# fishaudio/Bert-VITS2

Measured on AMD Instinct MI355X. Metric: audio-seconds/sec (44.1 kHz), SynthesizerTrn.infer(), 128-phoneme utterance, higher is better.
Workload: dtype f32; 1 GPU; BASELINE config 2: B=1 x T=128 symbols per GPU, fp32 Generator (split-bf16 MFMA), fp32 flow, fp32 text encoder / durations / spline; utterances_per_gpu=1, symbols=128, frames=384, parallelism=utterance-sharded x1, hipgraph=False, hip_force_dev_kernarg=1

## Files before the change

bert-vits2_amd/build.py:

```python
from __future__ import annotations

import hashlib
import os
import shutil
import subprocess
import sys

HERE = os.path.dirname(os.path.realpath(__file__))
CSRC = os.path.join(HERE, "csrc")
ROOT = os.path.dirname(HERE)
LIB = os.path.join(CSRC, "libbv2.so")
STAMP = os.path.join(CSRC, ".libbv2.stamp")

SOURCES = [
    "bv2_api.cpp", "bv2_model.cpp", "bv2_exec.cpp", "bv2_bert.cpp",
    "kernels/conv_mfma.hip", "kernels/conv_x6.hip", "kernels/respair_x6.hip", "kernels/resblock_fused.hip", "kernels/gen_bf16.hip", "kernels/resblock_cl_bf16.hip", "kernels/resblock_c16_bf16.hip", "kernels/respair_cl_bf16.hip", "kernels/enc_f16.hip", "kernels/layernorm.hip", "kernels/attention.hip", "kernels/misc.hip", "kernels/dds_fused.hip", "kernels/flow_boundary.hip", "kernels/bert.hip", "kernels/deberta_attn.hip", "kernels/ref_enc.hip", "kernels/stft.hip", "kernels/stream.hip",
]
EXPORTS = "libbv2.map"
HEADERS = [EXPORTS, "bv2_internal.h", "bv2_kernels.h", "kernels/spline.h", "kernels/cl_bf16.h", os.path.join(ROOT, "include", "bv2.h"),
           os.path.join(ROOT, "include", "bv2_testing.h"), os.path.join(ROOT, "include", "bv2_bert.h")]
FLAGS = ["--offload-arch=gfx950", "-O3", "-std=c++17", "-fPIC", "-Wall", "-Wno-unused-function", "-x", "hip"]


def _hipcc() -> str:
    for c in (os.environ.get("HIPCC"), shutil.which("hipcc"), "/opt/rocm/bin/hipcc"):
        if c and os.path.exists(c):
            return c
    raise RuntimeError("hipcc not found (need ROCm's hipcc to build libbv2.so for gfx950)")


def _digest() -> str:
# ... 53 lines not shown
```

bert-vits2_amd/csrc/bv2_api.cpp:

```cpp
#include <cmath>
#include <cstddef>
#include <cstring>
#include <functional>
#include <new>

#include "bv2_internal.h"

using namespace bv2;

static thread_local std::string g_create_err;

#define BV2_TRY try {
#define BV2_CATCH(h_)                                                                  \
  } catch (const std::exception& e) {                                                  \
    if (h_) (h_)->err = std::string("exception: ") + e.what();                         \
    return -100;                                                                       \
  } catch (...) {                                                                      \
    if (h_) (h_)->err = "unknown exception";                                           \
    return -100;                                                                       \
  }

extern "C" {

int bv2_abi_version(void) { return BV2_ABI_VERSION; }
// ... 28 lines not shown
  } catch (...) {
    delete h;
    g_create_err = "bv2_create: out of memory";
    return -100;
  }
  *out = h;
  return 0;
}

void bv2_destroy(bv2_handle* h) {
  if (!h) return;
  for (auto& r : h->prof_pool) { (void)hipEventDestroy(r.e0); (void)hipEventDestroy(r.e1); }
  if (h->ev_fork) (void)hipEventDestroy(h->ev_fork);
  if (h->ev_join) (void)hipEventDestroy(h->ev_join);
  if (h->side_stream) (void)hipStreamDestroy(h->side_stream);
  delete h;
}

const char* bv2_last_error(const bv2_handle* h) { return h ? h->err.c_str() : g_create_err.c_str(); }

static float half_to_float(uint16_t v) {
  const uint32_t sign = (uint32_t)(v & 0x8000) << 16;
  uint32_t exp = (v >> 10) & 0x1f, man = v & 0x3ff, bits;
  if (exp == 0) {
    if (man == 0) bits = sign;
    else {
      exp = 127 - 15 + 1;
      while (!(man & 0x400)) { man <<= 1; --exp; }
      man &= 0x3ff;
      bits = sign | (exp << 23) | (man << 13);
// ... 44 lines not shown
  uint32_t hdr[8];
  if (hipMemcpy(hdr, dev_blob, sizeof(hdr), hipMemcpyDeviceToHost) != hipSuccess) {
    h->err = "bv2_attach_weights: cannot read the blob header (is this a device pointer on the current GPU?)";
    return -6;
  }
  int64_t tf;
  std::memcpy(&tf, hdr + 4, sizeof(tf));
  if (hdr[0] != kBlobMagic || hdr[1] != BV2_ABI_VERSION || hdr[2] != h->model.cfg_hash || tf != h->model.total_floats) {
    h->err = "bv2_attach_weights: blob header does not match this handle's config (not packed, or packed for another model)";
    return -7;
  }
  if (hdr[3] != BV2_PACK_LAYOUT) {
    h->err = "bv2_attach_weights: blob was packed with another pack layout (a cache written by an older library build): repack";
    return -7;
  }
  h->blob = static_cast<const float*>(dev_blob);
  return 0;
  BV2_CATCH(h)
}

int bv2_detach_weights(bv2_handle* h) {
  if (!h) return -1;
  h->blob = nullptr;
  return 0;
}

int bv2_set_generator_dtype(bv2_handle* h, int dtype) {
  if (!h) return -1;
  if (dtype != BV2_F32 && dtype != BV2_BF16) { h->err = "bv2_set_generator_dtype: BV2_F32 or BV2_BF16"; return -1; }
  if (dtype == BV2_BF16) {
    const Model& m = h->model;
    bool ok = m.conv_pre.wb_off >= 0 && m.post_c % 8 == 0 && m.post_c <= 64;
    for (int i = 0; i < m.n_ups && ok; ++i) {
      ok = m.ups[i].cl.wb_off >= 0 && conv_cl_bf16_supported(m.ups[i].cl.cin, m.ups[i].cl.cout, m.ups[i].cl.k, 1);
      for (int j = 0; j < m.n_rbk && ok; ++j)
        for (int d = 0; d < m.n_rbd && ok; ++d)
          ok = m.rb[i][j][d][0].wb_off >= 0 &&
               conv_cl_bf16_supported(m.rb[i][j][d][0].cin, m.rb[i][j][d][0].cout, m.rb[i][j][d][0].k,
// ... 508 lines not shown
  if (!g) return;
  if (g->exec) (void)hipGraphExecDestroy(g->exec);
  delete g;
}

int bv2_set_option(bv2_handle* h, const char* key, int value) {
  if (!h) return -1;
  BV2_TRY
  const std::string k = key ? key : "";
  if (k == "fused_resblock") h->no_fused_resblock = value == 0;
  else if (k == "fused_respair") h->no_fused_respair = value == 0;
  else if (k == "fused_boundary") h->no_fused_boundary = value == 0;
  else if (k == "x6_pair") h->no_x6_pair = value == 0;
  else if (k == "x6_pair_c64") h->no_x6_pair_c64 = value == 0;
  else if (k == "x6_pair_c16") h->no_x6_pair_c16 = value == 0;
  else if (k == "x6_pair_c128") h->x6_pair_c128 = value != 0;
  else if (k == "respair_mix") h->respair_problem_major = value == 0;
  else if (k == "respair_form") h->respair_form = value;
  else if (k == "respair_c32") h->no_respair_c32 = value == 0;
  else if (k == "f16_wn") h->f16_wn = value;
  else if (k == "f16_ni") h->f16_ni = value;
  else if (k == "f16_kv") h->no_f16_kv = !value;
  else if (k == "stage_sum") h->no_stage_sum = !value;
  else if (k == "resblock_c16") h->no_resblock_c16 = value == 0;
  else if (k == "f16_fused_ln") h->no_f16_fused_ln = value == 0;
  else if (k == "f16_ksplit") h->no_f16_ksplit = value == 0;
  else if (k == "conv_post_rows") h->no_conv_post_rows = value == 0;
  else if (k == "ups_phase_taps") h->no_ups_phase_taps = value == 0;
  else if (k == "xcd_affine") h->no_xcd_affine = value == 0;
  else if (k == "prefetch") h->prefetch = value & 3;
// ... 385 lines not shown
    if (hipMemset(base, 0, boff + pb.size() * 4) != hipSuccess) return -6;
    if (hipMemcpy(base, pk.data(), pk.size() * 2, hipMemcpyHostToDevice) != hipSuccess) return -6;
    if (hipMemcpy(base + boff, pb.data(), pb.size() * 4, hipMemcpyHostToDevice) != hipSuccess) return -6;
    FusedLaunch F;
    std::memset(&F, 0, sizeof(F));
    F.nprob = 1; F.B = B; F.C = C; F.L = L; F.slope = slope; F.lens = lens; F.len_mul = 1;
    FusedProb& q = F.p[0];
    q.x = x; q.out = out; q.k = k; q.dil = dil;
    q.w61 = reinterpret_cast<const uint16_t*>(base); q.w62 = q.w61 + ne;
    q.b1 = reinterpret_cast<const float*>(base + boff); q.b2 = q.b1 + cout_pad;
    q.w1 = q.b1; q.w2 = q.b1;
    return launch_respair_x6(static_cast<hipStream_t>(stream), F);
  } catch (...) { return -100; }
}

int bv2_test_flow_boundary(void* stream, const float* a, int nslab, int64_t slab_stride, const float* gamma, const float* beta,
                           const float* mask, float* x1, int64_t z_bstride, const float* post_w_host, const float* post_b_host,
                           const float* pre_w_host, const float* pre_b_host, float* pre_out, float* wpack_dev, int B, int C, int T) {
  try {
    const int C1 = C / 2;
    const size_t npost = (size_t)t_round_up(C, 16) * t_round_up(C1, 128), npre = (size_t)t_round_up(C1, 16) * t_round_up(C, 128);
    std::vector<float> pk(npost + npre + (size_t)C1 + (size_t)C + 64, 0.f);
    for (int co = 0; co < C1; ++co)
      for (int ci = 0; ci < C; ++ci) pk[(size_t)conv_w_index(0, ci, co, t_round_up(C, 16), 1)] = post_w_host[(size_t)co * C + ci];
    if (pre_w_host)
      for (int co = 0; co < C; ++co)
        for (int ci = 0; ci < C1; ++ci) pk[npost + (size_t)conv_w_index(0, ci, co, t_round_up(C1, 16), 1)] = pre_w_host[(size_t)co * C1 + ci];
    for (int co = 0; co < C1; ++co) pk[npost + npre + co] = post_b_host[co];
    if (pre_b_host)
      for (int co = 0; co < C; ++co) pk[npost + npre + C1 + co] = pre_b_host[co];
// ... 253 lines not shown
```

bert-vits2_amd/csrc/bv2_exec.cpp:

```cpp
#include <cmath>
#include <cstdlib>
#include <cstring>

#include "bv2_internal.h"

namespace bv2 {

namespace {

struct Arena {
  char* base;
  int64_t off = 0, cap;
  Arena(void* b, int64_t c) : base(static_cast<char*>(b)), cap(c) {}
  template <class T> T* get(int64_t n) {
    const int64_t bytes = (n * (int64_t)sizeof(T) + 255) / 256 * 256;
    T* p = base ? reinterpret_cast<T*>(base + off) : nullptr;
    off += bytes;
    return p;
  }
  bool ok() const { return base == nullptr || off <= cap; }
};

struct Ctx {
  bv2_handle* h;
// ... 789 lines not shown
      hres = P.outacc;
    }
    {
      const std::string tn = "flow." + std::to_string(a) + ".enc";
      c.tap(tn.c_str(), hres, (int64_t)B * H * Ty);
    }
    p = c.prob(K.post, hres, x1, Ty);
    p.out_bstride = (int64_t)C * Ty; p.res = x1; p.res_bstride = (int64_t)C * Ty; p.res_mode = RES_RSUB;
    p.out_mask = ymask; p.mask_post = 1;
    c.conv1(p, B, Ty, "flow.post");
    {
      const std::string tn = "flow." + std::to_string(a) + ".z";
      c.tap(tn.c_str(), z, (int64_t)B * C * Ty);
    }
  }
}

static void gen_core(Ctx& c, const PlanB& P, const float* z, int z_rstride, const float* ymask, int B, int L, float* o,
                     const int64_t* lens) {
  const Model& m = c.m;
  const bv2_config& cf = m.cfg;
  const int C = cf.inter_channels, c0 = cf.upsample_initial_channel;
  {
    ConvProb p = c.prob(m.conv_pre, z, P.pre, L);
    p.x_bstride = (int64_t)C * z_rstride; p.x_rstride = z_rstride; p.Lin = L;
    p.in_mask = ymask; p.in_mask_bstride = z_rstride;
    p.bias2 = P.gv; p.bias2_bstride = P.gv_stride;
    c.conv1(p, B, L, "dec.conv_pre", 1, 0, lens, 1);
  }
  c.tap("dec.pre", P.pre, (int64_t)B * c0 * L);
// ... 57 lines not shown
        const bool to_cur = ((m.n_rbd - 1 - d) & 1) == 0;
        for (int jj = 0; jj < nb; ++jj) {
          const int j = nb - 1 - jj;
          float* cur = S[1 + j];
          float* tmp = S[1 + nb + j];
          const float* xin = d == 0 ? x : (to_cur ? tmp : cur);
          ConvProb p = c.prob(m.rb[i][j][d][0], xin, to_cur ? cur : tmp, Lo, cf.resblock_dilation_sizes[j][d]);
          p.pre_act = PRE_LRELU; p.slope = 0.1f;
          p.res = xin; p.res_mode = RES_ADD;
          p.w6 = (!c.h->no_conv_x6 && m.rb[i][j][d][0].wx_off >= 0) ? reinterpret_cast<const uint16_t*>(c.W(m.rb[i][j][d][0].wx_off)) : nullptr;
          c1.p[jj] = p;
        }
        c.conv(c1, "dec.resblock2.conv");
      }
      for (int j = 0; j < nb; ++j) branch_out[j] = S[1 + j];
    } else if (fused) {
      for (int j = 0; j < nb; ++j) branch_out[j] = nullptr;
      for (int d = 0; d < m.n_rbd; ++d) {
        FusedLaunch F;
        std::memset(&F, 0, sizeof(F));
        F.nprob = nb; F.B = B; F.C = U.cout; F.L = Lo; F.slope = 0.1f; F.lens = lens; F.len_mul = up * U.u;
        for (int jj = 0; jj < nb; ++jj) {
          const int j = nb - 1 - jj;
          float* a = S[1 + j];
          float* b2 = S[1 + nb + j];
          const float* xin = d == 0 ? x : branch_out[j];
          float* xout = (xin == a) ? b2 : a;
          FusedProb& p = F.p[jj];
          p.x = xin; p.out = xout;
          p.w1 = c.W(m.rb[i][j][d][0].w_off); p.b1 = c.W(m.rb[i][j][d][0].b_off);
// ... 487 lines not shown
```

bert-vits2_amd/csrc/bv2_internal.h:

```cpp
#pragma once
#include <hip/hip_runtime_api.h>
#include <stdint.h>

#include <map>
#include <string>
#include <vector>

#include "../../include/bv2.h"
#include "bv2_kernels.h"

namespace bv2 {

constexpr int kAttnWindow = 4;
constexpr int kCondLayer = 2;
constexpr int kSdpLayers = 3;
constexpr int kSdpKernel = 3;
constexpr int kSdpBins = 10;
constexpr int kSdpFlowsUsed = 3;
constexpr int kDpFilter = 256;
constexpr int kDpKernel = 3;
constexpr int kFlowKernel = 5;
constexpr int kMaxLayers = 16;
constexpr int kMaxFlows = 8;
constexpr uint32_t kBlobMagic = 0x32765642u;
// ... 65 lines not shown
  VecW dp_g1, dp_b1, dp_g2, dp_b2;
  VecW emb_g;
  RefEncW ref_enc;
  int n_coupling = 0;
  CouplingW coupling[kMaxFlows];
  ConvW conv_pre;
  GemvW dec_cond;
  int n_ups = 0, n_rbk = 0, n_rbd = 0;
  int rb_type = 1;
  UpW ups[BV2_MAX_UPS];
  ConvW rb[BV2_MAX_UPS][BV2_MAX_RESBLOCK_KERNELS][BV2_MAX_RESBLOCK_DILATIONS][2];
  int64_t rbcl_w_off[BV2_MAX_UPS][BV2_MAX_RESBLOCK_KERNELS];
  int64_t rbcl_b_off[BV2_MAX_UPS][BV2_MAX_RESBLOCK_KERNELS];
  int64_t rb16_w_off[BV2_MAX_UPS][BV2_MAX_RESBLOCK_KERNELS];
  int64_t rb16_b_off[BV2_MAX_UPS][BV2_MAX_RESBLOCK_KERNELS];
  VecW conv_post;
  int post_c = 0, post_k = 7;
  int total_up = 1;
  int64_t total_floats = 0;
  uint32_t cfg_hash = 0;
};

struct HostTensor { std::vector<float> data; std::vector<int64_t> shape; };

struct ProfileRec { hipEvent_t e0, e1; int fam; double flops, bytes; };

struct Tap { float* dst; int64_t cap; };

}

struct bv2_handle {
  bv2::Model model;
  std::map<std::string, bv2::HostTensor> tensors;
  const float* blob = nullptr;
  std::string err;
  std::map<std::string, bv2::Tap> taps;
  int gen_dtype = BV2_F32;
  int flow_dtype = BV2_F32;
  bool no_conv_x6 = false;
  bool no_conv_x3 = false;
  bool x6_narrow = true;
  bool no_fused_resblock = false;
  int prefetch = 0;
  bool no_xcd_affine = false;
  bool no_f16_fused_ln = false;
  int f16_wn = 0, f16_ni = 0;
  bool no_f16_kv = false;
  bool no_f16_ksplit = false;
  bool no_conv_post_rows = false;
  bool no_ups_phase_taps = false;
  bool no_stage_sum = true;
  bool no_resblock_c16 = false;
  bool no_respair_c32 = false;
  int respair_form = 1;
  bool respair_problem_major = false;
  bool x6_pair_c128 = false;
  bool no_x6_pair_c16 = false;
  bool no_x6_pair_c64 = false;
  bool no_x6_pair = false;
  bool no_fused_boundary = false;
  bool no_fused_respair = false;
  bool no_fused_attn_o = false;
  int attn_ksplit = -1;
  bool no_fused_dds = false;
  bool no_overlap_dp = true;
  hipStream_t side_stream = nullptr;
  hipEvent_t ev_fork = nullptr, ev_join = nullptr;
  bool prof_on = false;
  int prof_mode = 1;
  std::vector<bv2::ProfileRec> prof_pool;
  size_t prof_used = 0;
  std::vector<std::string> prof_names;
};

namespace bv2 {

int build_layout(Model& m, std::string& err);
int pack_blob(const Model& m, const std::map<std::string, HostTensor>& t, float* blob, std::string& err);
bool key_in_schema(const Model& m, const std::string& key);

int64_t workspace_bytes(const Model& m, int B, int T, int Ty);
int run_encode(bv2_handle* h, hipStream_t s, const bv2_encode_in& in, const bv2_encode_out& out, void* ws, int64_t wsb,
               const bv2_item_controls* ic = nullptr, const float* g_in = nullptr);
int run_ref_encode(bv2_handle* h, hipStream_t s, const float* y, const int64_t* strides, const int64_t* y_lengths, int B, int L,
                   float* g_out, void* ws, int64_t wsb);
int run_decode(bv2_handle* h, hipStream_t s, const bv2_decode_in& in, const bv2_decode_out& out, void* ws, int64_t wsb,
               const bv2_item_controls* ic = nullptr);
int run_flow(bv2_handle* h, hipStream_t s, int B, int Ty, const float* z_p, const int64_t* y_lengths, const float* y_mask,
             const float* g, float* z, void* ws, int64_t wsb);
int run_stage_emb_g(bv2_handle* h, hipStream_t s, int B, const int64_t* sid, float* g);
int run_stage_enc_p(bv2_handle* h, hipStream_t s, int B, int T, const int64_t* x, const int64_t* tone, const int64_t* lang,
                    const float* b0, const float* b1, const float* b2, const float* g, const int64_t* x_lengths, float* xout,
                    float* m_p, float* logs_p, float* x_mask, void* ws, int64_t wsb);
int run_stage_sdp(bv2_handle* h, hipStream_t s, int B, int T, const float* x, const float* x_mask, const float* zin,
// ... 14 lines not shown
```

bert-vits2_amd/csrc/bv2_kernels.h:

```cpp
#pragma once
#include <hip/hip_runtime_api.h>
#include <stdint.h>
#include <map>
#include <mutex>
#include <utility>

namespace bv2 {

#if defined(__HIPCC__)
__device__ __forceinline__ bool xcd_decode(unsigned id, int per, int B, int& b, int& r) {
  const unsigned slot = id >> 3;
  b = (int)(slot / (unsigned)per) * 8 + (int)(id & 7u);
  r = (int)(slot % (unsigned)per);
  return b < B;
}
#endif
inline int xcd_grid(int B, int per) { return 8 * ((B + 7) / 8) * per; }

struct Prefetch { const void* ptr; unsigned bytes; };
constexpr int PF_BLOCKS = 128;
#if defined(__HIPCC__)
__device__ __forceinline__ void prefetch_tail(const Prefetch pf, unsigned l, unsigned j, unsigned tid, unsigned nthreads) {
  const unsigned lines = (pf.bytes + 127u) >> 7;
  const unsigned lx = (lines + 7u) >> 3;
// ... 142 lines not shown
  const float* w1; const float* b1;
  const float* w2; const float* b2;
  int k, dil;
  const uint16_t* w61; const uint16_t* w62;
  const uint16_t* w31; const uint16_t* w32;
  const float* w3inv1; const float* w3inv2;
};
struct FusedLaunch { FusedProb p[3]; int nprob, B, C, L; float slope; const int64_t* lens = nullptr; int len_mul = 1;
                     unsigned long long* dbg = nullptr; };
bool resblock_fused_supported(int C, int k, int dil);
int launch_resblock_fused(hipStream_t stream, const FusedLaunch& F);
double resblock_fused_flops(const FusedLaunch& F);
double resblock_fused_bytes(const FusedLaunch& F);
bool respair_x6_supported(int C, int k, int dil);
int launch_respair_x6(hipStream_t stream, const FusedLaunch& F);

struct ClProb {
  const uint16_t* x[3];
  int nsrc; float in_scale;
  int64_t x_bstride;
  int Lin;
  const uint16_t* w;
  const float* bias;
  const float* bias2;
  int bias2_bstride;
  uint16_t* out;
  int64_t out_bstride;
  const uint16_t* res;
  int64_t res_bstride;
  int cin, cout, cout_pad, k, dil, pad_left;
// ... 297 lines not shown
```

bert-vits2_amd/csrc/bv2_model.cpp:

```cpp
#include <cmath>
#include <cstddef>
#include <cstring>
#include <functional>

#include "bv2_internal.h"

namespace bv2 {

static inline int round_up(int x, int m) { return (x + m - 1) / m * m; }

static inline uint16_t f2bf(float f) {
  uint32_t u;
  std::memcpy(&u, &f, 4);
  if ((u & 0x7fffffffu) > 0x7f800000u) return (uint16_t)((u >> 16) | 0x40u);
  u += 0x7fffu + ((u >> 16) & 1u);
  return (uint16_t)(u >> 16);
}

static inline uint16_t f2h(float f) {
  const _Float16 h = (_Float16)f;
  uint16_t u;
  std::memcpy(&u, &h, 2);
  return u;
}
// ... 311 lines not shown
          const float v = w[((int64_t)co * cin + ci) * 9 + t];
          if (i == 0) dst[t * 32 + co] = v;
          else dst[(((int64_t)(co / 8) * cin + ci) * 9 + t) * 8 + co % 8] = v;
        }
  }
  const int K = 128 * W[6];
  R.w_ih = P.vec("ref_enc.gru.weight_ih_l0", {384, K});
  R.w_hh = P.vec("ref_enc.gru.weight_hh_l0", {384, 128});
  R.b_ih = P.vec("ref_enc.gru.bias_ih_l0", {384});
  R.b_hh = P.vec("ref_enc.gru.bias_hh_l0", {384});
  R.pw = P.vec("ref_enc.proj.weight", {c.gin_channels, 128});
  R.pb = P.vec("ref_enc.proj.bias", {c.gin_channels});
}

int pack_all(Model& m, Packer& P) {
  const bv2_config& c = m.cfg;
  const int hid = c.hidden_channels, inter = c.inter_channels, filt = c.filter_channels, gin = c.gin_channels;
  const int half = inter / 2;

  m.emb = P.vec("enc_p.emb.weight", {c.n_vocab, hid});
  m.tone_emb = P.vec("enc_p.tone_emb.weight", {c.n_tones, hid});
  m.lang_emb = P.vec("enc_p.language_emb.weight", {c.n_languages, hid});
  const char* bn[3] = {"enc_p.bert_proj", "enc_p.ja_bert_proj", "enc_p.en_bert_proj"};
  for (int i = 0; i < 3; ++i) m.bert[i] = P.conv1d(bn[i], hid, c.bert_dim, 1);
  m.enc = pack_encoder(P, "enc_p.encoder", hid, filt, c.n_heads, c.n_layers, c.kernel_size, gin);
  m.proj_m = P.conv1d("enc_p.proj", 2 * inter, hid, 1, true, false, 0, inter);
  m.proj_logs = P.conv1d("enc_p.proj", 2 * inter, hid, 1, true, false, inter, inter);

  m.sdp_pre = P.conv1d("sdp.pre", hid, hid, 1);
  m.sdp_proj = P.conv1d("sdp.proj", hid, hid, 1);
// ... 111 lines not shown
      const std::string rp = "dec.resblocks." + std::to_string(i * m.n_rbk + j);
      P.emit_x6 = ch >= 16 && ch % 16 == 0;
      const bool rb2 = c.resblock_type == 2;
      for (int d = 0; d < m.n_rbd; ++d) {
        if (rb2) {
          m.rb[i][j][d][0] = P.conv1d(rp + ".convs." + std::to_string(d), ch, ch, k, true, true);
          m.rb[i][j][d][1] = ConvW();
        } else {
          m.rb[i][j][d][0] = P.conv1d(rp + ".convs1." + std::to_string(d), ch, ch, k, true, true);
          m.rb[i][j][d][1] = P.conv1d(rp + ".convs2." + std::to_string(d), ch, ch, k, true, true);
        }
      }
      P.emit_x6 = false;
      if (rb2) {
        m.rbcl_w_off[i][j] = m.rbcl_b_off[i][j] = m.rb16_w_off[i][j] = m.rb16_b_off[i][j] = -1;
        continue;
      }
      m.rbcl_w_off[i][j] = m.rbcl_b_off[i][j] = -1;
      if (m.n_rbd <= BV2_RBCL_MAX_D && resblock_cl_bf16_supported(ch, k, c.resblock_dilation_sizes[j], m.n_rbd)) {
        const int U = (ch / 16) * k, Upad = resblock_cl_bf16_units(ch, k);
        m.rbcl_w_off[i][j] = P.alloc(((int64_t)(2 * m.n_rbd * Upad + RBCL_PD) * 512 + 1) / 2);
        m.rbcl_b_off[i][j] = P.alloc((int64_t)2 * m.n_rbd * 32);
        if (P.fill()) {
          uint16_t* dst = reinterpret_cast<uint16_t*>(P.blob + m.rbcl_w_off[i][j]);
          for (int d = 0; d < m.n_rbd; ++d)
            for (int e = 0; e < 2; ++e) {
              const ConvW& cw = m.rb[i][j][d][e];
              const uint16_t* src = reinterpret_cast<const uint16_t*>(P.blob + cw.wb_off);
              const int G = ch / 16;
              for (int j2 = 0; j2 < k; ++j2)
// ... 12 lines not shown
        m.rb16_b_off[i][j] = P.alloc((int64_t)2 * m.n_rbd * 16);
        if (P.fill()) {
          uint16_t* dst = reinterpret_cast<uint16_t*>(P.blob + m.rb16_w_off[i][j]);
          std::memset(dst, 0, sizeof(uint16_t) * (size_t)2 * m.n_rbd * KU * 512);
          for (int d = 0; d < m.n_rbd; ++d)
            for (int e = 0; e < 2; ++e) {
              const ConvW& cw = m.rb[i][j][d][e];
              const uint16_t* src = reinterpret_cast<const uint16_t*>(P.blob + cw.wb_off);
              uint16_t* cd = dst + (int64_t)(2 * d + e) * KU * 512;
              for (int co = 0; co < 16; ++co)
                for (int ci = 0; ci < 16; ++ci)
                  for (int j2 = 0; j2 < k; ++j2) cd[rb16_w_index(j2, ci, co)] = src[cl_w_index(j2, ci, co, 16, k)];
              std::memcpy(P.blob + m.rb16_b_off[i][j] + (2 * d + e) * 16, P.blob + cw.b_off, sizeof(float) * 16);
            }
        }
      }
    }
  }
  P.emit_bf16 = false;
  m.post_c = ch;
  m.conv_post = P.vec("dec.conv_post.weight", {1, ch, m.post_k});
  P.alloc(2048);
  m.total_floats = P.cursor;
  return 0;
}

int validate(const bv2_config& c, std::string& err) {
  auto bad = [&](const char* s) { err = s; return -1; };
  auto in = [](int v, int lo, int hi) { return v >= lo && v <= hi; };
  if (c.struct_bytes != (int32_t)sizeof(bv2_config)) return bad("bv2_config.struct_bytes does not match this library");
// ... 53 lines not shown
  std::memset(blob, 0, sizeof(float) * kBlobHeaderFloats);
  pack_all(m, P);
  if (!P.missing.empty()) {
    err = "missing/invalid tensors (" + std::to_string(P.missing.size()) + "): ";
    for (size_t i = 0; i < P.missing.size() && i < 12; ++i) err += P.missing[i] + "; ";
    return -2;
  }
  if (m.total_floats != m_in.total_floats) { err = "internal: layout drift between passes"; return -4; }
  uint32_t* hdr = reinterpret_cast<uint32_t*>(blob);
  hdr[0] = kBlobMagic; hdr[1] = BV2_ABI_VERSION; hdr[2] = m_in.cfg_hash; hdr[3] = BV2_PACK_LAYOUT;
  int64_t tf = m.total_floats;
  std::memcpy(hdr + 4, &tf, sizeof(tf));
  return 0;
}

bool key_in_schema(const Model& m, const std::string& key) {
  (void)m;
  static const char* ignored[] = {"enc_q.", "sdp.post_", "sdp.flows.1."};
  for (const char* p : ignored)
    if (key.compare(0, std::strlen(p), p) == 0) return false;
  return true;
}

}
```

include/bv2_testing.h:

```cpp
#ifndef BV2_TESTING_H
#define BV2_TESTING_H
#include <stdint.h>
#include "bv2.h"
#ifdef __cplusplus
extern "C" {
#endif

int64_t bv2_test_conv_pack_floats(int cin, int cout, int k);

int bv2_test_conv1d(void* stream, const float* x, const float* w_host, const float* bias_host, float* out, float* wpack_dev,
                    int B, int cin, int cout, int k, int dil, int pad_left, int L, int tile, float lrelu_slope, int relu,
                    const float* res, int res_mode, const float* in_mask, const float* out_mask, int mask_pre,
                    int mask_post, const float* bias2, int nsrc, const float* x1, const float* x2, float in_scale, int ksplit,
                    int64_t slab_stride);


int64_t bv2_test_x3_omax_off(int cin, int cout, int k);

void bv2_test_x6_split(float v, uint16_t* h3);
int bv2_test_x6_regions(const bv2_handle* h, int64_t* off_floats, int64_t* n_floats, int max_regions);
int bv2_test_x3_regions(const bv2_handle* h, int64_t* off_floats, int64_t* n_floats, int max_regions);

int bv2_test_resblock_fused(void* stream, const float* x, float* out, const float* w1_host, const float* b1_host,
                            const float* w2_host, const float* b2_host, float* wpack_dev, int B, int C, int k, int dil, int L,
// ... 4 lines not shown
                          const float* bias_host, void* wpack_dev, void* out, const void* res, const float* bias2, int B, int cin,
                          int cout, int k, int dil, int pad_left, int L, int pre_lrelu, float slope);

int64_t bv2_test_resblock_cl_pack_bytes(int C, int k, int nd);
int bv2_test_resblock_cl(void* stream, const void* x, void* out, const float* w_host, const float* bias_host, void* wpack_dev, int B,
                         int C, int k, const int* dil, int nd, int L, float slope, int variant, const int64_t* lens);

int64_t bv2_test_respair_cl_pack_bytes(int C, int k);
int bv2_test_respair_cl(void* stream, const void* x, void* out, const float* w_host, const float* bias_host, void* wpack_dev, int B,
                        int C, int k, int dil, int L, float slope, int form, const int64_t* lens);
int64_t bv2_test_respair_x6_pack_bytes(int C, int k);
int bv2_test_respair_x6(void* stream, const float* x, float* out, const float* w_host, const float* bias_host, void* wpack_dev, int B,
                        int C, int k, int dil, int L, float slope, const int64_t* lens);
int bv2_test_respair_x3(void* stream, const float* x, float* out, const float* w_host, const float* bias_host, void* wpack_dev, int B,
                        int C, int k, int dil, int L, float slope, const int64_t* lens);
int64_t bv2_test_flow_boundary_pack_floats(int C);
int bv2_test_flow_boundary(void* stream, const float* a, int nslab, int64_t slab_stride, const float* gamma, const float* beta,
                           const float* mask, float* x1, int64_t z_bstride, const float* post_w_host, const float* post_b_host,
                           const float* pre_w_host, const float* pre_b_host, float* pre_out, float* wpack_dev, int B, int C, int T);

int bv2_test_conv_f16(void* stream, const void* x, int in_ct, const float* in_mask, const float* w_host, const float* bias_host,
                      void* wpack_dev, void* out, int out_ct, const float* res, int res_mode, const float* out_mask, int mask_pre,
                      int mask_post, int act, int B, int cin, int cout, int k, int dil, int L, int out_rstride);

int bv2_test_dump_cl_conv(bv2_handle* h, const void* host_blob, int kind, int i, int j, int d, int e, int32_t* dims,
                          float* w_out, float* bias_out);

int bv2_test_attention(void* stream, const float* qkv, int ld, const float* mask, const float* erv, float* out,
                       int B, int H, int D, int T, int W);
int bv2_test_attention_f16(void* stream, const float* qkv, int ld, const float* mask, const float* erv, float* out,
// ... 30 lines not shown
```

Baseline: 1443 audio-seconds/sec.

## Fuse whole C=16 resblock stage into one split-f16 MFMA kernel

Adds a resstage_x3 kernel that runs every dilation layer of every resblock branch at the final C=16 generator stage in a single launch. Each block keeps its tile in registers and LDS across the layers and recomputes halos instead of writing intermediates between layer pairs. Activations are rescaled per tile and multiplied against split-f16 weight planes. Those planes are rebuilt into a side buffer on the device when weights are attached. This removes several launches and the global round trips of intermediates on a long-sequence stage, at the cost of redundant halo compute and extra attach-time work and memory.

```diff
diff --git a/bert-vits2_amd/build.py b/bert-vits2_amd/build.py
--- a/bert-vits2_amd/build.py
+++ b/bert-vits2_amd/build.py
@@ -14,7 +14,7 @@
 
 SOURCES = [
     "bv2_api.cpp", "bv2_model.cpp", "bv2_exec.cpp", "bv2_bert.cpp",
-    "kernels/conv_mfma.hip", "kernels/conv_x6.hip", "kernels/respair_x6.hip", "kernels/resblock_fused.hip", "kernels/gen_bf16.hip", "kernels/resblock_cl_bf16.hip", "kernels/resblock_c16_bf16.hip", "kernels/respair_cl_bf16.hip", "kernels/enc_f16.hip", "kernels/layernorm.hip", "kernels/attention.hip", "kernels/misc.hip", "kernels/dds_fused.hip", "kernels/flow_boundary.hip", "kernels/bert.hip", "kernels/deberta_attn.hip", "kernels/ref_enc.hip", "kernels/stft.hip", "kernels/stream.hip",
+    "kernels/conv_mfma.hip", "kernels/conv_x6.hip", "kernels/respair_x6.hip", "kernels/resstage_x3.hip", "kernels/resblock_fused.hip", "kernels/gen_bf16.hip", "kernels/resblock_cl_bf16.hip", "kernels/resblock_c16_bf16.hip", "kernels/respair_cl_bf16.hip", "kernels/enc_f16.hip", "kernels/layernorm.hip", "kernels/attention.hip", "kernels/misc.hip", "kernels/dds_fused.hip", "kernels/flow_boundary.hip", "kernels/bert.hip", "kernels/deberta_attn.hip", "kernels/ref_enc.hip", "kernels/stft.hip", "kernels/stream.hip",
 ]
 EXPORTS = "libbv2.map"
 HEADERS = [EXPORTS, "bv2_internal.h", "bv2_kernels.h", "kernels/spline.h", "kernels/cl_bf16.h", os.path.join(ROOT, "include", "bv2.h"),
diff --git a/bert-vits2_amd/csrc/bv2_api.cpp b/bert-vits2_amd/csrc/bv2_api.cpp
--- a/bert-vits2_amd/csrc/bv2_api.cpp
+++ b/bert-vits2_amd/csrc/bv2_api.cpp
@@ -66,6 +66,7 @@
   if (h->ev_fork) (void)hipEventDestroy(h->ev_fork);
   if (h->ev_join) (void)hipEventDestroy(h->ev_join);
   if (h->side_stream) (void)hipStreamDestroy(h->side_stream);
+  if (h->rs3_dev) (void)hipFree(h->rs3_dev);
   delete h;
 }
 
@@ -140,6 +141,19 @@
     h->err = "bv2_attach_weights: blob was packed with another pack layout (a cache written by an older library build): repack";
     return -7;
   }
+  if (h->rs3_dev) { (void)hipFree(h->rs3_dev); h->rs3_dev = nullptr; }
+  if (h->model.rs3_floats > 0) {
+    std::vector<float> side((size_t)h->model.rs3_floats);
+    const float* db = static_cast<const float*>(dev_blob);
+    const int rc = rs3_fill(h->model, [&](int64_t off, int64_t n, float* dst) {
+      return hipMemcpy(dst, db + off, sizeof(float) * (size_t)n, hipMemcpyDeviceToHost) == hipSuccess ? 0 : -6; }, side.data());
+    if (rc || hipMalloc(reinterpret_cast<void**>(&h->rs3_dev), side.size() * sizeof(float)) != hipSuccess ||
+        hipMemcpy(h->rs3_dev, side.data(), side.size() * sizeof(float), hipMemcpyHostToDevice) != hipSuccess) {
+      if (h->rs3_dev) { (void)hipFree(h->rs3_dev); h->rs3_dev = nullptr; }
+      h->err = "bv2_attach_weights: cannot build the C = 16 stage's tap-pair weight planes on the device";
+      return -6;
+    }
+  }
   h->blob = static_cast<const float*>(dev_blob);
   return 0;
   BV2_CATCH(h)
@@ -148,6 +162,7 @@
 int bv2_detach_weights(bv2_handle* h) {
   if (!h) return -1;
   h->blob = nullptr;
+  if (h->rs3_dev) { (void)hipFree(h->rs3_dev); h->rs3_dev = nullptr; }
   return 0;
 }
 
@@ -686,6 +701,7 @@
   else if (k == "x6_pair") h->no_x6_pair = value == 0;
   else if (k == "x6_pair_c64") h->no_x6_pair_c64 = value == 0;
   else if (k == "x6_pair_c16") h->no_x6_pair_c16 = value == 0;
+  else if (k == "resstage_x3") h->no_resstage_x3 = value == 0;
   else if (k == "x6_pair_c128") h->x6_pair_c128 = value != 0;
   else if (k == "respair_mix") h->respair_problem_major = value == 0;
   else if (k == "respair_form") h->respair_form = value;
@@ -1101,6 +1117,85 @@
   } catch (...) { return -100; }
 }
 
+int64_t bv2_test_resstage_x3_pack_bytes(const int* ks, int nb, int nd) {
+  int64_t n = 0;
+  for (int j = 0; j < nb; ++j) n += x3r_w_elems(ks[j], nd) * 2 + (int64_t)2 * nd * 16 * 4 + 256;
+  return n + 256;
+}
+int bv2_test_resstage_x3(void* stream, const float* x, float* out, const float* w_host, const float* bias_host, void* wpack_dev, int B,
+                         const int* ks, const int* dils, int nb, int nd, int L, float slope, const int64_t* lens, int len_mul) {
+  try {
+    if (nb < 1 || nb > 3 || nd < 1 || nd > BV2_STAGE_MAX_D || !resstage_x3_supported(16, ks, dils, nd, nd, nb)) return -2;
+    std::vector<char> pk((size_t)bv2_test_resstage_x3_pack_bytes(ks, nb, nd), 0);
+    StageLaunch F;
+    std::memset(&F, 0, sizeof(F));
+    F.nprob = nb; F.B = B; F.C = 16; F.L = L; F.nd = nd; F.slope = slope; F.lens = lens; F.len_mul = len_mul;
+    size_t cur = 0, wsrc = 0;
+    char* base = static_cast<char*>(wpack_dev);
+    for (int j = 0; j < nb; ++j) {
+      const int k = ks[j], KU = x3r_units(k);
+      uint16_t* wd = reinterpret_cast<uint16_t*>(pk.data() + cur);
+      const size_t woff = cur;
+      cur += (size_t)x3r_w_elems(k, nd) * 2;
+      float* bd = reinterpret_cast<float*>(pk.data() + cur);
+      const size_t boff = cur;
+      cur += (size_t)2 * nd * 16 * 4;
+      float* id = reinterpret_cast<float*>(pk.data() + cur);
+      const size_t ioff = cur;
+      cur += 256;
+      for (int c = 0; c < 2 * nd; ++c) {
+        const float* w = w_host + wsrc + (size_t)c * 256 * k;
+        float wmax = 0.f;
+        for (int i = 0; i < 256 * k; ++i) wmax = std::max(wmax, std::fabs(w[i]));
+        uint32_t mb;
+        std::memcpy(&mb, &wmax, 4);
+        const unsigned ex = x3_scale_exp(mb);
+        id[c] = x3_scale_inv(ex);
+        for (int co = 0; co < 16; ++co)
+          for (int ci = 0; ci < 16; ++ci)
+            for (int t = 0; t < k; ++t) {
+              const float v = w[((size_t)co * 16 + ci) * k + t] * x3_scale(ex);
+              const _Float16 g0 = (_Float16)v;
+              const _Float16 g1 = (_Float16)(v - (float)g0);
+              std::memcpy(&wd[(size_t)c * KU * 1024 + (size_t)x3r_w_index(t, ci, co, 0)], &g0, 2);
+              std::memcpy(&wd[(size_t)c * KU * 1024 + (size_t)x3r_w_index(t, ci, co, 1)], &g1, 2);
+            }
+        for (int co = 0; co < 16; ++co) bd[c * 16 + co] = bias_host[((size_t)j * 2 * nd + c) * 16 + co];
+      }
+      wsrc += (size_t)2 * nd * 256 * k;
+      StageProb& q = F.p[j];
+      q.x = x; q.out = out + (size_t)j * B * 16 * L; q.k = k;
+      for (int d = 0; d < nd; ++d) q.dil[d] = dils[j * nd + d];
+      q.w = reinterpret_cast<const uint16_t*>(base + woff);
+      q.bias = reinterpret_cast<const float*>(base + boff);
+      q.winv = reinterpret_cast<const float*>(base + ioff);
+    }
+    if (hipMemcpy(base, pk.data(), pk.size(), hipMemcpyHostToDevice) != hipSuccess) return -6;
+    return launch_resstage_x3(static_cast<hipStream_t>(stream), F);
+  } catch (...) { return -100; }
+}
+int64_t bv2_test_x3r_floats(const bv2_handle* h) { return h ? h->model.rs3_floats : -1; }
+int bv2_test_x3r_build(const bv2_handle* h, const void* host_blob, float* side_out) {
+  if (!h || !host_blob || !side_out) return -1;
+  try {
+    const float* hb = static_cast<const float*>(host_blob);
+    return rs3_fill(h->model, [&](int64_t off, int64_t n, float* dst) { std::memcpy(dst, hb + off, sizeof(float) * (size_t)n); return 0; }, side_out);
+  } catch (...) { return -100; }
+}
+int bv2_test_x3r_conv(const bv2_handle* h, int i, int j, int d, int e, int64_t* off_floats, int64_t* inv_off_floats, int64_t* bias_off_floats,
+                      int64_t* x3_off_floats, int* k) {
+  if (!h || !off_floats || !inv_off_floats || !bias_off_floats || !x3_off_floats || !k) return -1;
+  const Model& m = h->model;
+  if (i < 0 || i >= m.n_ups || j < 0 || j >= m.n_rbk || d < 0 || d >= m.n_rbd || (e != 0 && e != 1) || m.rs3_w_off[i][j] < 0) return -2;
+  const ConvW& w = m.rb[i][j][d][e];
+  *k = w.k;
+  *off_floats = m.rs3_w_off[i][j] + (int64_t)(2 * d + e) * x3r_units(w.k) * 512;
+  *inv_off_floats = m.rs3_i_off[i][j] + 2 * d + e;
+  *bias_off_floats = m.rs3_b_off[i][j] + (2 * d + e) * 16;
+  *x3_off_floats = w.wy_off;
+  return 0;
+}
+
 int bv2_test_flow_boundary(void* stream, const float* a, int nslab, int64_t slab_stride, const float* gamma, const float* beta,
                            const float* mask, float* x1, int64_t z_bstride, const float* post_w_host, const float* post_b_host,
                            const float* pre_w_host, const float* pre_b_host, float* pre_out, float* wpack_dev, int B, int C, int T) {
diff --git a/bert-vits2_amd/csrc/bv2_exec.cpp b/bert-vits2_amd/csrc/bv2_exec.cpp
--- a/bert-vits2_amd/csrc/bv2_exec.cpp
+++ b/bert-vits2_amd/csrc/bv2_exec.cpp
@@ -827,6 +827,15 @@
       c.tap(tn.c_str(), z, (int64_t)B * C * Ty);
     }
   }
+}
+
+static bool stage_x3_ok(const Ctx& c, int i) {
+  const Model& m = c.m;
+  const bv2_config& cf = m.cfg;
+  if (m.ups[i].cout != 16 || c.h->no_resstage_x3 || c.h->no_conv_x3 || !c.h->taps.empty() || m.n_rbd > BV2_STAGE_MAX_D || !c.h->rs3_dev) return false;
+  for (int j = 0; j < m.n_rbk; ++j)
+    if (m.rs3_w_off[i][j] < 0 || m.rs3_b_off[i][j] < 0 || m.rs3_i_off[i][j] < 0) return false;
+  return resstage_x3_supported(16, cf.resblock_kernel_sizes, &cf.resblock_dilation_sizes[0][0], BV2_MAX_RESBLOCK_DILATIONS, m.n_rbd, m.n_rbk);
 }
 
 static void gen_core(Ctx& c, const PlanB& P, const float* z, int z_rstride, const float* ymask, int B, int L, float* o,
@@ -914,6 +923,29 @@
         c.conv(c1, "dec.resblock2.conv");
       }
       for (int j = 0; j < nb; ++j) branch_out[j] = S[1 + j];
+    } else if (x6pair && stage_x3_ok(c, i)) {
+      StageLaunch F;
+      std::memset(&F, 0, sizeof(F));
+      F.nprob = nb; F.B = B; F.C = U.cout; F.L = Lo; F.nd = m.n_rbd; F.slope = 0.1f; F.lens = lens; F.len_mul = up * U.u;
+      for (int jj = 0; jj < nb; ++jj) {
+        const int j = nb - 1 - jj;
+        StageProb& p = F.p[jj];
+        p.x = x; p.out = S[1 + j];
+        p.w = reinterpret_cast<const uint16_t*>(c.h->rs3_dev + m.rs3_w_off[i][j]);
+        p.bias = c.h->rs3_dev + m.rs3_b_off[i][j]; p.winv = c.h->rs3_dev + m.rs3_i_off[i][j];
+        p.k = cf.resblock_kernel_sizes[j];
+        for (int d = 0; d < m.n_rbd; ++d) p.dil[d] = cf.resblock_dilation_sizes[j][d];
+        branch_out[j] = S[1 + j];
+      }
+      if (!c.rc) {
+        const int pi = c.prof_begin("dec.resblock.stage");
+        if (pi >= 0 && c.h->prof_mode >= 3)
+          c.cur_shape = " n" + std::to_string(nb) + " C" + std::to_string(U.cout) + " k" + std::to_string(F.p[0].k) + " L" + std::to_string(Lo) +
+                        " B" + std::to_string(B);
+        const int r = launch_resstage_x3(c.s, F);
+        c.prof_end(pi, "resstage_x3<16>", resstage_x3_flops(F), resstage_x3_bytes(F));
+        if (r) c.fail("dec.resblock.stage", r);
+      }
     } else if (fused) {
       for (int j = 0; j < nb; ++j) branch_out[j] = nullptr;
       for (int d = 0; d < m.n_rbd; ++d) {
diff --git a/bert-vits2_amd/csrc/bv2_internal.h b/bert-vits2_amd/csrc/bv2_internal.h
--- a/bert-vits2_amd/csrc/bv2_internal.h
+++ b/bert-vits2_amd/csrc/bv2_internal.h
@@ -1,4 +1,5 @@
 #pragma once
+#include <functional>
 #include <hip/hip_runtime_api.h>
 #include <stdint.h>
 
@@ -103,6 +104,10 @@
   int64_t rbcl_b_off[BV2_MAX_UPS][BV2_MAX_RESBLOCK_KERNELS];
   int64_t rb16_w_off[BV2_MAX_UPS][BV2_MAX_RESBLOCK_KERNELS];
   int64_t rb16_b_off[BV2_MAX_UPS][BV2_MAX_RESBLOCK_KERNELS];
+  int64_t rs3_floats = 0;
+  int64_t rs3_w_off[BV2_MAX_UPS][BV2_MAX_RESBLOCK_KERNELS];
+  int64_t rs3_b_off[BV2_MAX_UPS][BV2_MAX_RESBLOCK_KERNELS];
+  int64_t rs3_i_off[BV2_MAX_UPS][BV2_MAX_RESBLOCK_KERNELS];
   VecW conv_post;
   int post_c = 0, post_k = 7;
   int total_up = 1;
@@ -122,6 +127,7 @@
   bv2::Model model;
   std::map<std::string, bv2::HostTensor> tensors;
   const float* blob = nullptr;
+  float* rs3_dev = nullptr;
   std::string err;
   std::map<std::string, bv2::Tap> taps;
   int gen_dtype = BV2_F32;
@@ -144,6 +150,7 @@
   int respair_form = 1;
   bool respair_problem_major = false;
   bool x6_pair_c128 = false;
+  bool no_resstage_x3 = false;
   bool no_x6_pair_c16 = false;
   bool no_x6_pair_c64 = false;
   bool no_x6_pair = false;
@@ -167,6 +174,7 @@
 int build_layout(Model& m, std::string& err);
 int pack_blob(const Model& m, const std::map<std::string, HostTensor>& t, float* blob, std::string& err);
 bool key_in_schema(const Model& m, const std::string& key);
+int rs3_fill(const Model& m, const std::function<int(int64_t, int64_t, float*)>& read, float* side);
 
 int64_t workspace_bytes(const Model& m, int B, int T, int Ty);
 int run_encode(bv2_handle* h, hipStream_t s, const bv2_encode_in& in, const bv2_encode_out& out, void* ws, int64_t wsb,
diff --git a/bert-vits2_amd/csrc/bv2_kernels.h b/bert-vits2_amd/csrc/bv2_kernels.h
--- a/bert-vits2_amd/csrc/bv2_kernels.h
+++ b/bert-vits2_amd/csrc/bv2_kernels.h
@@ -180,6 +180,22 @@
 double resblock_fused_bytes(const FusedLaunch& F);
 bool respair_x6_supported(int C, int k, int dil);
 int launch_respair_x6(hipStream_t stream, const FusedLaunch& F);
+
+#define BV2_STAGE_MAX_D 4
+inline int x3r_units(int k) { return (k + 1) / 2; }
+inline int64_t x3r_w_index(int j, int ci, int co, int plane) {
+  const int q = 2 * (j & 1) + (ci >> 3);
+  return (((int64_t)(j >> 1) * 2 + plane) * 64 + co + 16 * q) * 8 + (ci & 7);
+}
+inline int64_t x3r_w_elems(int k, int nd) { return (int64_t)2 * nd * x3r_units(k) * 1024; }
+struct StageProb { const float* x; float* out; const uint16_t* w; const float* winv; const float* bias; int k; int dil[BV2_STAGE_MAX_D]; int halo; };
+struct StageLaunch { StageProb p[3]; int nprob, B, C, L, nd; float slope; const int64_t* lens = nullptr; int len_mul = 1; };
+bool resstage_x3_branch_supported(int C, int k, const int* dil, int nd);
+bool resstage_x3_supported(int C, const int* ks, const int* dils, int dil_stride, int nd, int nb);
+int resstage_x3_halo(int k, const int* dil, int nd);
+int launch_resstage_x3(hipStream_t stream, const StageLaunch& L);
+double resstage_x3_flops(const StageLaunch& L);
+double resstage_x3_bytes(const StageLaunch& L);
 
 struct ClProb {
   const uint16_t* x[3];
diff --git a/bert-vits2_amd/csrc/bv2_model.cpp b/bert-vits2_amd/csrc/bv2_model.cpp
--- a/bert-vits2_amd/csrc/bv2_model.cpp
+++ b/bert-vits2_amd/csrc/bv2_model.cpp
@@ -349,6 +349,7 @@
 }
 
 int pack_all(Model& m, Packer& P) {
+  m.rs3_floats = 0;
   const bv2_config& c = m.cfg;
   const int hid = c.hidden_channels, inter = c.inter_channels, filt = c.filter_channels, gin = c.gin_channels;
   const int half = inter / 2;
@@ -490,6 +491,7 @@
       P.emit_x6 = false;
       if (rb2) {
         m.rbcl_w_off[i][j] = m.rbcl_b_off[i][j] = m.rb16_w_off[i][j] = m.rb16_b_off[i][j] = -1;
+        m.rs3_w_off[i][j] = m.rs3_b_off[i][j] = m.rs3_i_off[i][j] = -1;
         continue;
       }
       m.rbcl_w_off[i][j] = m.rbcl_b_off[i][j] = -1;
@@ -532,6 +534,15 @@
               std::memcpy(P.blob + m.rb16_b_off[i][j] + (2 * d + e) * 16, P.blob + cw.b_off, sizeof(float) * 16);
             }
         }
+      }
+      m.rs3_w_off[i][j] = m.rs3_b_off[i][j] = m.rs3_i_off[i][j] = -1;
+      bool rs3 = m.n_rbd <= BV2_STAGE_MAX_D && resstage_x3_branch_supported(ch, k, c.resblock_dilation_sizes[j], m.n_rbd);
+      for (int d = 0; d < m.n_rbd && rs3; ++d) rs3 = m.rb[i][j][d][0].wy_off >= 0 && m.rb[i][j][d][1].wy_off >= 0;
+      if (rs3) {
+        auto side = [&](int64_t n) { const int64_t off = m.rs3_floats; m.rs3_floats += (n + 63) / 64 * 64; return off; };
+        m.rs3_w_off[i][j] = side((x3r_w_elems(k, m.n_rbd) + 1) / 2);
+        m.rs3_b_off[i][j] = side((int64_t)2 * m.n_rbd * 16);
+        m.rs3_i_off[i][j] = side((int64_t)2 * m.n_rbd);
       }
     }
   }
@@ -615,6 +626,32 @@
   return 0;
 }
 
+int rs3_fill(const Model& m, const std::function<int(int64_t, int64_t, float*)>& read, float* side) {
+  std::memset(side, 0, sizeof(float) * (size_t)m.rs3_floats);
+  std::vector<float> reg;
+  for (int i = 0; i < m.n_ups; ++i)
+    for (int j = 0; j < m.n_rbk; ++j) {
+      if (m.rs3_w_off[i][j] < 0) continue;
+      for (int d = 0; d < m.n_rbd; ++d)
+        for (int e = 0; e < 2; ++e) {
+          const ConvW& cw = m.rb[i][j][d][e];
+          const int k = cw.k;
+          const int64_t nreg = X3_HDR_FLOATS + (x3_w_elems(16, 32, k) + 1) / 2;
+          reg.resize((size_t)nreg);
+          if (int rc = read(cw.wy_off, nreg, reg.data())) return rc;
+          if (int rc = read(cw.b_off, 16, side + m.rs3_b_off[i][j] + (2 * d + e) * 16)) return rc;
+          side[m.rs3_i_off[i][j] + 2 * d + e] = reg[0];
+          const uint16_t* src = reinterpret_cast<const uint16_t*>(reg.data() + X3_HDR_FLOATS);
+          uint16_t* cd = reinterpret_cast<uint16_t*>(side + m.rs3_w_off[i][j]) + (int64_t)(2 * d + e) * x3r_units(k) * 1024;
+          for (int co = 0; co < 16; ++co)
+            for (int ci = 0; ci < 16; ++ci)
+              for (int j2 = 0; j2 < k; ++j2)
+                for (int pl = 0; pl < 2; ++pl) cd[x3r_w_index(j2, ci, co, pl)] = src[x3_w_index(j2, ci, co, 16, k, pl)];
+        }
+    }
+  return 0;
+}
+
 bool key_in_schema(const Model& m, const std::string& key) {
   (void)m;
   static const char* ignored[] = {"enc_q.", "sdp.post_", "sdp.flows.1."};
diff --git a/bert-vits2_amd/csrc/kernels/resstage_x3.hip b/bert-vits2_amd/csrc/kernels/resstage_x3.hip
--- /dev/null
+++ b/bert-vits2_amd/csrc/kernels/resstage_x3.hip
@@ -0,0 +1,300 @@
+#include <hip/hip_runtime.h>
+#include "../bv2_kernels.h"
+
+namespace bv2 {
+
+namespace {
+
+typedef _Float16 sxf16x8 __attribute__((ext_vector_type(8)));
+typedef _Float16 sxf16x2 __attribute__((ext_vector_type(2)));
+typedef float sxf32x2 __attribute__((ext_vector_type(2)));
+typedef float sxf32x4 __attribute__((ext_vector_type(4)));
+typedef unsigned sxu32x2 __attribute__((ext_vector_type(2)));
+typedef unsigned sxu32x4 __attribute__((ext_vector_type(4)));
+typedef __attribute__((address_space(1))) sxf16x8 SxGlobalFrag;
+
+constexpr int SX_G = 32;
+constexpr int SX_NW = 8;
+constexpr int SX_NB = 8;
+constexpr int SX_R = 16 * SX_NB * SX_NW;
+constexpr int SX_ROWS = SX_R + 2 * SX_G;
+constexpr unsigned SX_ROWB = 32;
+constexpr unsigned SX_PLANE = SX_ROWS * SX_ROWB;
+constexpr unsigned SX_BLK = 16 * SX_ROWB;
+constexpr int SX_PAIR_HT = 256;
+
+extern __shared__ __attribute__((aligned(16))) unsigned short sx_lds[];
+__device__ __forceinline__ float sx_ld(const float* base, unsigned byte_off) {
+  return *reinterpret_cast<const float*>(reinterpret_cast<const char*>(base) + byte_off);
+}
+__device__ __forceinline__ void sx_st(float* base, unsigned byte_off, float v) {
+  *reinterpret_cast<float*>(reinterpret_cast<char*>(base) + byte_off) = v;
+}
+__device__ __forceinline__ sxf16x8 sx_rd128(unsigned off) {
+  return *reinterpret_cast<const sxf16x8*>(reinterpret_cast<const char*>(sx_lds) + off);
+}
+__device__ __forceinline__ void sx_wr64(unsigned off, sxu32x2 v) {
+  *reinterpret_cast<sxu32x2*>(reinterpret_cast<char*>(sx_lds) + off) = v;
+}
+__device__ __forceinline__ void sx_split2h(float a, float b, unsigned& u1, unsigned& u2) {
+  const sxf16x2 g = __builtin_convertvector((sxf32x2){a, b}, sxf16x2);
+  const sxf32x2 f = __builtin_convertvector(g, sxf32x2);
+  u1 = __builtin_bit_cast(unsigned, g);
+  u2 = __builtin_bit_cast(unsigned, __builtin_convertvector((sxf32x2){a - f[0], b - f[1]}, sxf16x2));
+}
+__device__ __forceinline__ void sx_wave_max_to(float* red, int wid, int lane, float m) {
+  asm volatile("" : "+v"(lane));
+#pragma unroll
+  for (int d = 32; d >= 1; d >>= 1)
+    m = fmaxf(m, __int_as_float(__builtin_amdgcn_ds_bpermute((lane ^ d) << 2, __float_as_int(m))));
+  if (lane == 0) red[wid] = m;
+}
+__device__ __forceinline__ float sx_wg_max(const float* red) {
+  float M = red[0];
+#pragma unroll
+  for (int w = 1; w < SX_NW; ++w) M = fmaxf(M, red[w]);
+  return M;
+}
+
+template <int KU>
+__device__ __forceinline__ void sx_gemm(sxf32x4 (&acc)[SX_NB], const uint16_t* w, unsigned wl, unsigned rd0, unsigned ustep) {
+  sxf16x8 W[2][2];
+  const char* const wb = reinterpret_cast<const char*>(w);
+#pragma unroll
+  for (int p = 0; p < 2; ++p) W[0][p] = *(const SxGlobalFrag*)(wb + 1024 * p + wl);
+#pragma unroll
+  for (int nb = 0; nb < SX_NB; ++nb) acc[nb] = sxf32x4{0.f, 0.f, 0.f, 0.f};
+#pragma unroll
+  for (int u = 0; u < KU; ++u) {
+    if (u + 1 < KU) {
+#pragma unroll
+      for (int p = 0; p < 2; ++p) W[(u + 1) & 1][p] = *(const SxGlobalFrag*)(wb + 2048 * (u + 1) + 1024 * p + wl);
+    }
+    const unsigned xb = rd0 + (unsigned)u * ustep;
+#pragma unroll
+    for (int nb = 0; nb < SX_NB; nb += 2) {
+      sxf16x8 b0[2], b1[2];
+#pragma unroll
+      for (int i = 0; i < 2; ++i) {
+        b0[i] = sx_rd128(xb + (nb + i) * SX_BLK);
+        b1[i] = sx_rd128(SX_PLANE + xb + (nb + i) * SX_BLK);
+      }
+#pragma unroll
+      for (int i = 0; i < 2; ++i) acc[nb + i] = __builtin_amdgcn_mfma_f32_16x16x32_f16(W[u & 1][1], b0[i], acc[nb + i], 0, 0, 0);
+#pragma unroll
+      for (int i = 0; i < 2; ++i) acc[nb + i] = __builtin_amdgcn_mfma_f32_16x16x32_f16(W[u & 1][0], b1[i], acc[nb + i], 0, 0, 0);
+#pragma unroll
+      for (int i = 0; i < 2; ++i) acc[nb + i] = __builtin_amdgcn_mfma_f32_16x16x32_f16(W[u & 1][0], b0[i], acc[nb + i], 0, 0, 0);
+      __builtin_amdgcn_sched_barrier(0);
+    }
+  }
+}
+
+__device__ __forceinline__ void sx_store_planes(unsigned own, const float (&v)[4], int ni) {
+  unsigned a1, a2, c1, c2;
+  sx_split2h(v[0], v[1], a1, a2);
+  sx_split2h(v[2], v[3], c1, c2);
+  sx_wr64(own + ni * SX_BLK, sxu32x2{a1, c1});
+  sx_wr64(SX_PLANE + own + ni * SX_BLK, sxu32x2{a2, c2});
+}
+
+template <int KU>
+__device__ __forceinline__ void sx_block(const StageLaunch& L, const StageProb& P, int b, int t0, int TT, int Lin, int E) {
+  constexpr int NT = 64 * SX_NW;
+  const int tid = threadIdx.x, lane = tid & 63;
+  const int wid = __builtin_amdgcn_readfirstlane(tid >> 6);
+  const int t = lane & 15, q = lane >> 4, row0 = wid * 16 * SX_NB;
+  const int hk = (P.k - 1) / 2, nd = L.nd;
+  const int base = t0 - P.halo;
+  int tg0 = base + row0 + t;
+  unsigned own = (unsigned)((SX_G + row0 + t) * SX_ROWB + 8 * q);
+  unsigned rd = (unsigned)((SX_G + row0 + t) * SX_ROWB + (q & 1) * 16);
+  const int qt = q >> 1;
+  const unsigned wl = 16u * (unsigned)lane;
+  const float slope = L.slope;
+  float* const red = reinterpret_cast<float*>(reinterpret_cast<char*>(sx_lds) + 2 * SX_PLANE);
+  const unsigned Lrow = (unsigned)L.L;
+  const float* const xg = P.x + (int64_t)b * 16 * L.L;
+  float* const og = P.out + (int64_t)b * 16 * L.L;
+
+  float xr[SX_NB][4];
+#pragma unroll
+  for (int ni = 0; ni < SX_NB; ++ni) {
+    const int tg = tg0 + 16 * ni;
+    const unsigned tc = (unsigned)(tg < 0 ? 0 : (tg >= L.L ? L.L - 1 : tg));
+#pragma unroll
+    for (int i = 0; i < 4; ++i) xr[ni][i] = sx_ld(xg, 4u * ((unsigned)(4 * q + i) * Lrow + tc));
+  }
+  for (int p = tid; p < 4 * SX_G; p += NT) {
+    const int gr = p >> 1, pc = p & 1;
+    const int row = gr < SX_G ? gr : SX_R + gr;
+    const unsigned off = (unsigned)row * SX_ROWB + 16u * (unsigned)pc;
+    *reinterpret_cast<sxu32x4*>(reinterpret_cast<char*>(sx_lds) + off) = sxu32x4{0u, 0u, 0u, 0u};
+    *reinterpret_cast<sxu32x4*>(reinterpret_cast<char*>(sx_lds) + SX_PLANE + off) = sxu32x4{0u, 0u, 0u, 0u};
+  }
+
+  int M = 0;
+  for (int d = 0; d < nd; ++d) {
+    const int dil = P.dil[d];
+    asm volatile("" : "+v"(tg0), "+v"(own), "+v"(rd));
+    const uint16_t* const w1 = P.w + (int64_t)(2 * d) * KU * 1024;
+    const int xlo = base + M > 0 ? base + M : 0, xhi = base + SX_R - M < Lin ? base + SX_R - M : Lin;
+    float mx = 0.f;
+#pragma unroll
+    for (int ni = 0; ni < SX_NB; ++ni) {
+      const int tg = tg0 + 16 * ni;
+      const bool ok = tg >= xlo && tg < xhi;
+#pragma unroll
+      for (int i = 0; i < 4; ++i) mx = fmaxf(mx, ok ? fabsf(xr[ni][i]) : 0.f);
+    }
+    sx_wave_max_to(red, wid, lane, mx);
+    __syncthreads();
+    const unsigned ex = x3_scale_exp(__float_as_uint(sx_wg_max(red)));
+    const float Sx = x3_scale(ex);
+    const float s1 = x3_scale_inv(ex) * P.winv[2 * d];
+#pragma unroll
+    for (int ni = 0; ni < SX_NB; ++ni) {
+      const int tg = tg0 + 16 * ni;
+      const bool ok = tg >= xlo && tg < xhi;
+      float v[4];
+#pragma unroll
+      for (int i = 0; i < 4; ++i) {
+        float a = xr[ni][i];
+        const float an = a * slope;
+        a = a < 0.f ? an : a;
+        v[i] = ok ? a * Sx : 0.f;
+      }
+      sx_store_planes(own, v, ni);
+    }
+    __syncthreads();
+
+    sxf32x4 acc[SX_NB];
+    sx_gemm<KU>(acc, w1, wl, rd + (unsigned)((qt - hk) * dil * (int)SX_ROWB), (unsigned)(2 * dil) * SX_ROWB);
+
+    const int hlo = base + M + hk * dil > 0 ? base + M + hk * dil : 0;
+    const int hhi = base + SX_R - M - hk * dil < Lin ? base + SX_R - M - hk * dil : Lin;
+    asm volatile("" : "+v"(tg0), "+v"(own), "+v"(rd));
+    const sxf32x4 b1v = *reinterpret_cast<const sxf32x4*>(reinterpret_cast<const char*>(P.bias + (2 * d) * 16) + 16u * (unsigned)q);
+    float mh = 0.f;
+#pragma unroll
+    for (int ni = 0; ni < SX_NB; ++ni) {
+      const int tg = tg0 + 16 * ni;
+      const bool ok = tg >= hlo && tg < hhi;
+#pragma unroll
+      for (int i = 0; i < 4; ++i) {
+        float tt = __builtin_fmaf(acc[ni][i], s1, b1v[i]);
+        const float tn = tt * slope;
+        tt = tt < 0.f ? tn : tt;
+        tt = ok ? tt : 0.f;
+        acc[ni][i] = tt;
+        mh = fmaxf(mh, fabsf(tt));
+      }
+    }
+    sx_wave_max_to(red + SX_NW, wid, lane, mh);
+    __syncthreads();
+    const unsigned eh = x3_scale_exp(__float_as_uint(sx_wg_max(red + SX_NW)));
+    const float Sh = x3_scale(eh);
+    const float s2 = x3_scale_inv(eh) * P.winv[2 * d + 1];
+#pragma unroll
+    for (int ni = 0; ni < SX_NB; ++ni) {
+      float v[4];
+#pragma unroll
+      for (int i = 0; i < 4; ++i) v[i] = acc[ni][i] * Sh;
+      sx_store_planes(own, v, ni);
+    }
+    const sxf32x4 b2v = *reinterpret_cast<const sxf32x4*>(reinterpret_cast<const char*>(P.bias + (2 * d + 1) * 16) + 16u * (unsigned)q);
+    __syncthreads();
+
+    sx_gemm<KU>(acc, w1 + (int64_t)KU * 1024, wl, rd + (unsigned)((qt - hk) * (int)SX_ROWB), 2u * SX_ROWB);
+
+#pragma unroll
+    for (int ni = 0; ni < SX_NB; ++ni)
+#pragma unroll
+      for (int i = 0; i < 4; ++i) xr[ni][i] = __builtin_fmaf(acc[ni][i], s2, b2v[i]) + xr[ni][i];
+    M += hk * (dil + 1);
+  }
+
+  const int tend = t0 + TT < E ? t0 + TT : E;
+#pragma unroll
+  for (int ni = 0; ni < SX_NB; ++ni) {
+    const int tg = tg0 + 16 * ni;
+    if (tg >= t0 && tg < tend) {
+#pragma unroll
+      for (int i = 0; i < 4; ++i) sx_st(og, 4u * ((unsigned)(4 * q + i) * Lrow + (unsigned)tg), xr[ni][i]);
+    }
+  }
+}
+
+}
+
+__global__ void __launch_bounds__(64 * SX_NW, 4) resstage_x3_kernel(const StageLaunch L) {
+  const StageProb& P = L.p[blockIdx.z];
+  const int TT = SX_R - 2 * P.halo;
+  const int t0 = blockIdx.x * TT;
+  if (t0 >= L.L) return;
+  const int b = blockIdx.y;
+  int Lin = L.L;
+  if (L.lens) {
+    const int64_t lv = L.lens[b] * L.len_mul;
+    Lin = __builtin_amdgcn_readfirstlane(lv < L.L ? (int)lv : L.L);
+  }
+  const int BTp = SX_PAIR_HT - (P.k - 1);
+  int E = Lin > 0 ? ((Lin - 1) / BTp + 1) * BTp : 0;
+  E = E < L.L ? E : L.L;
+  if (t0 >= E) return;
+  switch (P.k) {
+    case 3: sx_block<2>(L, P, b, t0, TT, Lin, E); break;
+    case 5: sx_block<3>(L, P, b, t0, TT, Lin, E); break;
+    case 7: sx_block<4>(L, P, b, t0, TT, Lin, E); break;
+    case 9: sx_block<5>(L, P, b, t0, TT, Lin, E); break;
+    default: sx_block<6>(L, P, b, t0, TT, Lin, E); break;
+  }
+}
+
+int resstage_x3_halo(int k, const int* dil, int nd) {
+  int h = 0;
+  for (int d = 0; d < nd; ++d) h += (k - 1) / 2 * (dil[d] + 1);
+  return h;
+}
+
+bool resstage_x3_branch_supported(int C, int k, const int* dil, int nd) {
+  if (C != 16) return false;
+  if (k < 3 || k > 11 || k % 2 == 0 || nd < 1 || nd > BV2_STAGE_MAX_D) return false;
+  for (int d = 0; d < nd; ++d)
+    if (dil[d] < 1 || ((k + 1) / 2) * dil[d] > SX_G) return false;
+  return 8 * resstage_x3_halo(k, dil, nd) <= SX_R;
+}
+
+bool resstage_x3_supported(int C, const int* ks, const int* dils, int dil_stride, int nd, int nb) {
+  if (nb < 1 || nb > 3) return false;
+  for (int j = 0; j < nb; ++j)
+    if (!resstage_x3_branch_supported(C, ks[j], dils + (int64_t)j * dil_stride, nd)) return false;
+  return true;
+}
+
+int launch_resstage_x3(hipStream_t stream, const StageLaunch& L0) {
+  StageLaunch L = L0;
+  if (L.nprob < 1 || L.nprob > 3 || L.B < 1 || L.L < 1 || L.C != 16 || (int64_t)L.L * 16 >= (1ll << 29)) return -1;
+  int max_tiles = 0;
+  for (int i = 0; i < L.nprob; ++i) {
+    StageProb& p = L.p[i];
+    if (!resstage_x3_branch_supported(L.C, p.k, p.dil, L.nd) || !p.x || !p.out || p.x == p.out || !p.w || !p.winv || !p.bias) return -1;
+    p.halo = resstage_x3_halo(p.k, p.dil, L.nd);
+    const int TT = SX_R - 2 * p.halo;
+    const int nt = (L.L + TT - 1) / TT;
+    if (nt > max_tiles) max_tiles = nt;
+  }
+  const size_t lds = (size_t)2 * SX_PLANE + 2 * SX_NW * sizeof(float);
+  ensure_dyn_lds((const void*)resstage_x3_kernel, lds);
+  hipLaunchKernelGGL(resstage_x3_kernel, dim3(max_tiles, L.B, L.nprob), dim3(64 * SX_NW), lds, stream, L);
+  return hipGetLastError() == hipSuccess ? 0 : -1;
+}
+
+double resstage_x3_flops(const StageLaunch& L) {
+  double f = 0;
+  for (int i = 0; i < L.nprob; ++i) f += 2.0 * L.nd * 2.0 * 16 * 16 * L.p[i].k * (double)L.L * L.B;
+  return f;
+}
+double resstage_x3_bytes(const StageLaunch& L) { return 2.0 * L.nprob * 16.0 * (double)L.L * L.B * 4.0; }
+
+}
diff --git a/include/bv2_testing.h b/include/bv2_testing.h
--- a/include/bv2_testing.h
+++ b/include/bv2_testing.h
@@ -42,6 +42,13 @@
                         int C, int k, int dil, int L, float slope, const int64_t* lens);
 int bv2_test_respair_x3(void* stream, const float* x, float* out, const float* w_host, const float* bias_host, void* wpack_dev, int B,
                         int C, int k, int dil, int L, float slope, const int64_t* lens);
+int64_t bv2_test_resstage_x3_pack_bytes(const int* ks, int nb, int nd);
+int bv2_test_resstage_x3(void* stream, const float* x, float* out, const float* w_host, const float* bias_host, void* wpack_dev, int B,
+                         const int* ks, const int* dils, int nb, int nd, int L, float slope, const int64_t* lens, int len_mul);
+int64_t bv2_test_x3r_floats(const bv2_handle* h);
+int bv2_test_x3r_build(const bv2_handle* h, const void* host_blob, float* side_out);
+int bv2_test_x3r_conv(const bv2_handle* h, int i, int j, int d, int e, int64_t* off_floats, int64_t* inv_off_floats, int64_t* bias_off_floats,
+                      int64_t* x3_off_floats, int* k);
 int64_t bv2_test_flow_boundary_pack_floats(int C);
 int bv2_test_flow_boundary(void* stream, const float* a, int nslab, int64_t slab_stride, const float* gamma, const float* beta,
                            const float* mask, float* x1, int64_t z_bstride, const float* post_w_host, const float* post_b_host,
```

Result: no change. 1460 audio-seconds/sec (median of 6 runs) (+1.2%).
